# wyhuai/DDNM

Measured on AMD Instinct MI355X. Metric: restored images/sec @256×256, 100 DDIM steps, 4×SR; 1/2/4/8 GPU, higher is better.
Workload: dtype f32 (3x3 convolutions: fp32 operands carried as hi + lo fp16 halves, three fp16 MFMA products per product, fp32 accumulate -- operand error 2^-22, measured closer to fp64 than the fp32 MFMA kernel; everything else fp32); 1 GPU; celeba_hq.yml SVD sr_bicubic 4x, sigma_y=0, eta=0.85, T_sampling=100, batch_size=8 per GPU (BASELINE configs[1]); global_batch=8, image=3x256x256, parallelism=dp1 (image sharding)

## Files before the change

### ddnm_amd/_lib.py

```python
import ctypes
import os
from ctypes import POINTER, Structure, c_char_p, c_float, c_int32, c_int64, c_uint32, c_void_p

_HERE = os.path.dirname(os.path.abspath(__file__))
LIB_PATH = os.path.join(_HERE, "libddnm_hip.so")

c_f32p = c_void_p


class ConvDesc(Structure):
    _fields_ = [
        ("src0", c_void_p), ("src1", c_void_p), ("weight", c_void_p), ("bias", c_void_p),
        ("badd", c_void_p), ("res", c_void_p), ("gn_scale", c_void_p), ("gn_shift", c_void_p),
        ("out", c_void_p),
        ("B", c_int32), ("Hin", c_int32), ("Win", c_int32),
        ("C0", c_int32), ("C1", c_int32), ("Cout", c_int32),
        ("ksize", c_int32), ("stride", c_int32), ("pad", c_int32),
        ("Ho", c_int32), ("Wo", c_int32),
        ("ups", c_int32), ("gn_silu", c_int32), ("out_nchw", c_int32),
        ("badd_stride", c_int32), ("tile", c_int32),
        ("workspace", c_void_p), ("workspace_floats", c_int64),
        ("res_ups", c_int32), ("src_f16", c_int32),
        ("stats_out", c_void_p),
        ("skip0", c_void_p), ("skip1", c_void_p), ("skip_weight", c_void_p),
# ... 39 lines not shown
    _fields_ = [("sqrt_1m_at", c_float), ("sqrt_at", c_float), ("sqrt_at_next", c_float),
                ("c1", c_float), ("c2", c_float), ("lam", c_float),
                ("rng_on", c_uint32), ("rng_seed_lo", c_uint32), ("rng_seed_hi", c_uint32), ("rng_iter", c_uint32),
                ("rng_image_base", c_uint32), ("reserved_rng", c_uint32)]


PROTOTYPES = {
    "ddnm_version": (c_int32, []),
    "ddnm_error_string": (c_char_p, [c_int32]),
    "ddnm_build_digest": (c_char_p, []),
    "ddnm_sizeof": (c_int32, [c_int32]),
    "ddnm_conv2d_f32": (c_int32, [POINTER(ConvDesc), c_void_p]),
    "ddnm_conv3x3_small_cout_f32": (c_int32, [POINTER(ConvDesc), c_void_p]),
    "ddnm_conv3x3_small_cout_f32_supported": (c_int32, [POINTER(ConvDesc)]),
    "ddnm_conv2d_f32_tile_n": (c_int32, [POINTER(ConvDesc)]),
    "ddnm_conv2d_f32_workspace_floats": (c_int64, [POINTER(ConvDesc)]),
    "ddnm_conv2d_f32_stats_tiles": (c_int32, [POINTER(ConvDesc)]),
    "ddnm_conv2d_f32_fuses_skip": (c_int32, [POINTER(ConvDesc)]),
    "ddnm_spectral_mix_f32": (c_int32, [c_void_p, c_void_p, c_void_p, c_int64, c_void_p, c_int64, c_float, c_float, c_float,
                                        c_float, c_int32, c_void_p]),
    "ddnm_hq_x0_f32": (c_int32, [c_void_p, c_void_p, c_int64, c_void_p, c_int32, c_int64, c_float, c_float, c_int32,
                                 c_void_p]),
    "ddnm_hq_project_f32": (c_int32, [c_void_p, c_void_p, c_void_p, c_void_p, c_int64, c_float, c_void_p]),
    "ddnm_copy_rect_f32": (c_int32, [c_void_p, c_int32, c_int32, c_int32, c_int32, c_void_p, c_int32, c_int32, c_int32,
                                     c_int32, c_int32, c_int32, c_int32, c_void_p]),
    "ddnm_hq_sample_f32": (c_int32, [c_void_p, c_void_p, c_void_p, c_void_p, c_void_p, c_int64, c_float, c_float, c_float,
                                     c_float, c_void_p]),
    "ddnm_patchify_f32": (c_int32, [c_void_p, c_void_p, c_int32, c_int32, c_int32, c_int32, c_void_p]),
    "ddnm_im2col3x3_f16": (c_int32, [c_void_p, c_void_p, c_void_p, c_void_p, c_void_p, c_int32, c_int32, c_int32, c_int32,
                                     c_int32, c_int32, c_void_p]),
    "ddnm_gn_apply_f16": (c_int32, [c_void_p, c_void_p, c_void_p, c_void_p, c_void_p, c_int32, c_int32, c_int32, c_int32,
                                    c_int32, c_void_p]),
    "ddnm_gn_finalize_tiles_f32": (c_int32, [c_void_p, c_int32, c_int32, c_void_p, c_int32, c_int32, c_void_p, c_void_p,
                                             c_int32, c_int32, c_int32, c_float, c_void_p, c_void_p, c_void_p, c_int32,
                                             c_void_p, c_void_p]),
    "ddnm_gn_finalize_tiles_amax_f32": (c_int32, [c_void_p, c_int32, c_int32, c_void_p, c_int32, c_int32, c_void_p, c_void_p,
                                                  c_int32, c_int32, c_int32, c_float, c_void_p, c_void_p, c_void_p, c_int32,
                                                  c_void_p, c_void_p, c_void_p]),
    "ddnm_amax_bound_f32": (c_int32, [c_void_p, c_int64, c_int32, c_void_p, c_int64, c_int32, c_void_p, c_int32, c_void_p]),
    "ddnm_conv3x3_f16_f32": (c_int32, [POINTER(ConvDesc), c_void_p]),
    "ddnm_conv3x3_f16_supported": (c_int32, [POINTER(ConvDesc)]),
    "ddnm_conv3x3_f16_workspace_floats": (c_int64, [POINTER(ConvDesc)]),
    "ddnm_conv3x3_f16_stats_tiles": (c_int32, [POINTER(ConvDesc)]),
    "ddnm_conv3x3_s16_f32": (c_int32, [POINTER(ConvDesc), c_void_p]),
    "ddnm_conv3x3_s16_supported": (c_int32, [POINTER(ConvDesc)]),
    "ddnm_conv3x3_s16_persistent": (c_int32, [POINTER(ConvDesc)]),
    "ddnm_conv3x3_s16_workspace_floats": (c_int64, [POINTER(ConvDesc)]),
    "ddnm_conv3x3_s16_stats_tiles": (c_int32, [POINTER(ConvDesc)]),
    "ddnm_conv3x3_s16_act_scale": (c_float, []),
    "ddnm_conv_gather_s16_f32": (c_int32, [POINTER(ConvDesc), c_void_p]),
    "ddnm_conv_gather_s16_supported": (c_int32, [POINTER(ConvDesc)]),
    "ddnm_conv_gather_s16_workspace_floats": (c_int64, [POINTER(ConvDesc)]),
    "ddnm_conv_gather_s16_stats_tiles": (c_int32, [POINTER(ConvDesc)]),
    "ddnm_conv16": (c_int32, [POINTER(Conv16Desc), c_void_p]),
    "ddnm_conv16_supported": (c_int32, [POINTER(Conv16Desc)]),
    "ddnm_conv16_fuses_fin": (c_int32, [POINTER(Conv16Desc)]),
    "ddnm_conv16_workspace_floats": (c_int64, [POINTER(Conv16Desc)]),
    "ddnm_conv16_stats_tiles": (c_int32, [POINTER(Conv16Desc)]),
    "ddnm_gn_apply_h16": (c_int32, [c_void_p, c_void_p, c_void_p, c_void_p, c_void_p, c_int32, c_int32, c_int32, c_int32,
                                    c_int32, c_int32, c_int32, c_void_p]),
    "ddnm_im2col3x3_h16": (c_int32, [c_void_p, c_void_p, c_void_p, c_void_p, c_void_p, c_int32, c_int32, c_int32, c_int32,
                                     c_int32, c_int32, c_void_p]),
    "ddnm_nchw_to_nhwc_h16": (c_int32, [c_void_p, c_void_p, c_int32, c_int32, c_int32, c_int32, c_void_p]),
    "ddnm_gn_stats_h16": (c_int32, [c_void_p, c_void_p, c_int32, c_int32, c_int32, c_int32, c_void_p]),
    "ddnm_attn16_d64": (c_int32, [c_void_p, c_void_p, c_int32, c_int32, c_int32, c_void_p]),
    "ddnm_conv1x1_f16_f32": (c_int32, [POINTER(ConvDesc), c_void_p]),
    "ddnm_conv1x1_f16_supported": (c_int32, [POINTER(ConvDesc)]),
    "ddnm_conv1x1_f16_workspace_floats": (c_int64, [POINTER(ConvDesc)]),
    "ddnm_conv1x1_f16_stats_tiles": (c_int32, [POINTER(ConvDesc)]),
    "ddnm_gn_stats_f32": (c_int32, [c_void_p, c_void_p, c_int32, c_int32, c_int32, c_int32, c_int32, c_void_p,
                                    c_int32, c_void_p]),
    "ddnm_gn_nchunk": (c_int32, [c_int32, c_int32]),
    "ddnm_gn_finalize_f32": (c_int32, [c_void_p, c_int32, c_void_p, c_void_p, c_int32, c_int32, c_int32, c_int32,
                                       c_float, c_void_p, c_void_p, c_void_p, c_int32, c_void_p, c_void_p]),
    "ddnm_bgemm_f32": (c_int32, [POINTER(GemmDesc), c_void_p]),
    "ddnm_gn_bwd_f32": (c_int32, [c_void_p, c_void_p, c_int32, c_void_p, c_void_p, c_void_p, c_int32, c_void_p, c_int32,
                                  c_int32, c_int32, c_int32, c_int32, c_int32, c_void_p, c_int32, c_void_p, c_void_p,
                                  c_void_p]),
    "ddnm_gn_bwd_nchunk": (c_int32, [c_int32, c_int32]),
    "ddnm_gn_bwd_h16": (c_int32, [c_void_p, c_void_p, c_int32, c_void_p, c_void_p, c_void_p, c_int32, c_void_p, c_int32,
                                  c_int32, c_int32, c_int32, c_int32, c_int32, c_void_p, c_int32, c_void_p, c_void_p,
                                  c_void_p]),
    "ddnm_pool_tokens_h16": (c_int32, [c_void_p, c_void_p, c_void_p, c_void_p, c_void_p, c_int32, c_int32, c_int32,
                                       c_void_p]),
    "ddnm_pool_tokens_bwd_h16": (c_int32, [c_void_p, c_void_p, c_int32, c_int32, c_int32, c_void_p]),
    "ddnm_attn16_d64_lse": (c_int32, [c_void_p, c_void_p, c_void_p, c_int32, c_int32, c_int32, c_void_p]),
    "ddnm_attn16_d64_bwd": (c_int32, [c_void_p, c_void_p, c_void_p, c_void_p, c_void_p, c_void_p, c_int32, c_int32,
                                      c_int32, c_void_p]),
    "ddnm_softmax_bwd_rows_f32": (c_int32, [c_void_p, c_void_p, c_int64, c_int32, c_int32, c_float, c_void_p]),
    "ddnm_pool_tokens_f32": (c_int32, [c_void_p, c_void_p, c_void_p, c_void_p, c_void_p, c_int32, c_int32, c_int32,
                                       c_void_p]),
    "ddnm_pool_attn_fwd_f32": (c_int32, [c_void_p, c_void_p, c_void_p, c_int32, c_int32, c_int32, c_int32, c_void_p]),
    "ddnm_pool_attn_bwd_f32": (c_int32, [c_void_p, c_void_p, c_void_p, c_void_p, c_int32, c_int32, c_int32, c_int32,
                                         c_void_p]),
    "ddnm_pool_tokens_bwd_f32": (c_int32, [c_void_p, c_void_p, c_int32, c_int32, c_int32, c_void_p]),
    "ddnm_logsoftmax_grad_f32": (c_int32, [c_void_p, c_void_p, c_void_p, c_int32, c_int32, c_void_p]),
    "ddnm_softmax_rows_f32": (c_int32, [c_void_p, c_int64, c_int32, c_int32, c_float, c_void_p]),
    "ddnm_linear_f32": (c_int32, [c_void_p, c_void_p, c_void_p, c_void_p, c_int32, c_int32, c_int32, c_int32,
                                  c_void_p]),
    "ddnm_timestep_embedding_f32": (c_int32, [c_void_p, c_void_p, c_void_p, c_int32, c_int32, c_int32, c_void_p]),
    "ddnm_avgpool2_nhwc_f32": (c_int32, [c_void_p, c_void_p, c_void_p, c_int32, c_void_p, c_int32, c_int32, c_int32,
                                         c_int32, c_void_p]),
    "ddnm_embedding_add_f32": (c_int32, [c_void_p, c_void_p, c_void_p, c_int32, c_int32, c_int32, c_void_p]),
    "ddnm_nchw_im2col3x3_pad_f32": (c_int32, [c_void_p, c_void_p, c_int32, c_int32, c_int32, c_int32, c_int32, c_void_p]),
    "ddnm_nchw_to_nhwc_pad_f32": (c_int32, [c_void_p, c_void_p, c_int32, c_int32, c_int32, c_int32, c_void_p]),
    "ddnm_step_x0_f32": (c_int32, [c_void_p, c_void_p, c_int64, c_void_p, c_int32, c_int64, POINTER(StepScalars),
# ... 103 lines not shown
```

### ddnm_amd/build.py

```python
import hashlib
import os
import shutil
import subprocess
import sys

HERE = os.path.dirname(os.path.abspath(__file__))
CSRC = os.path.join(HERE, "csrc")
LIB = os.path.join(HERE, "libddnm_hip.so")
STAMP = os.path.join(HERE, ".libddnm_hip.stamp")
OBJ = os.path.join(HERE, "_obj")
SOURCES = ["conv_igemm_f32.hip", "conv_igemm_f16.hip", "conv_s16_persist.hip", "conv_gather_s16.hip", "conv_small_f32.hip", "conv1x1_f16.hip", "conv16.hip", "act16.hip", "attn16.hip", "attn_d512.hip", "attn16_bwd.hip", "gemm_f32.hip", "groupnorm.hip", "misc.hip", "ddnm_step.hip", "fwht.hip", "backward.hip"]
FLAGS = ["--offload-arch=gfx950", "-O3", "-std=c++17", "-fPIC", "-shared", "-Wall", "-Wno-unused-function"]


def _hipcc():
    for c in (os.environ.get("HIPCC"), shutil.which("hipcc"), "/opt/rocm/bin/hipcc"):
        if c and os.path.exists(c):
            return c
    raise RuntimeError("hipcc not found (set HIPCC)")


def _digest():
    h = hashlib.sha256()
    for f in sorted(os.listdir(CSRC)) + ["../../include/ddnm_hip.h"]:
        with open(os.path.join(CSRC, f), "rb") as fh:
            h.update(f.encode() + fh.read())
    h.update(" ".join(FLAGS).encode())
    return h.hexdigest()


LAST_BUILD = {"compiled": False}


def build(force=False, verbose=False):
    dig = _digest()
    LAST_BUILD["compiled"] = False
    if not force and os.path.exists(LIB) and os.path.exists(STAMP) and open(STAMP).read() == dig:
        return LIB
    LAST_BUILD["compiled"] = True
    tmp = LIB + f".tmp{os.getpid()}"
    os.makedirs(OBJ, exist_ok=True)
    hh = hashlib.sha256()
    for f in sorted(os.listdir(CSRC)) + ["../../include/ddnm_hip.h"]:
        if f.endswith(".h"):
            with open(os.path.join(CSRC, f), "rb") as fh:
                hh.update(f.encode() + fh.read())
    hh.update(" ".join(FLAGS).encode())
    cflags = [f for f in FLAGS if f != "-shared"]
    jobs, objs = [], []
    for s in SOURCES:
        h = hashlib.sha256(hh.digest())
        with open(os.path.join(CSRC, s), "rb") as fh:
            h.update(fh.read())
        extra = [f'-DDDNM_BUILD_DIGEST="{dig}"'] if s == "misc.hip" else []
        h.update(" ".join(extra).encode())
        obj = os.path.join(OBJ, f"{s}.{h.hexdigest()[:16]}.o")
        objs.append(obj)
        if force or not os.path.exists(obj):
            jobs.append((s, [_hipcc()] + cflags + extra + ["-c", os.path.join(CSRC, s), "-o", obj + f".tmp{os.getpid()}"], obj))
    if jobs:
        from concurrent.futures import ThreadPoolExecutor

        def run(job):
            s, cmd, obj = job
# ... 34 lines not shown
```

### ddnm_amd/csrc/conv_common.h

```cpp
#pragma once
#include "common.h"

struct ConvArgs {
    ddnm_conv_desc d;
    int Cin, ntaps, Hs, Ws;
    int m_tiles, n_tiles;
    int tiles_x;
    int TW, TW_log2;
    int ksplit;
    float* ws;
};

static inline bool conv_sizes_addressable(const ddnm_conv_desc* d) {
    const int64_t lim = (int64_t)1 << 31;
    const int64_t out_el = (int64_t)d->B * d->Ho * d->Wo * d->Cout;
    const int64_t hs = d->ups ? d->Hin / 2 : d->Hin, ws = d->ups ? d->Win / 2 : d->Win;
    const int64_t cmax = d->C0 > d->C1 ? d->C0 : d->C1;
    const int64_t src_b = (int64_t)d->B * hs * ws * cmax * (d->src_f16 ? 2 : 4);
    const int64_t cout_pad = ((int64_t)d->Cout + 127) / 128 * 128;
    const int64_t w_b = cout_pad * d->ksize * d->ksize * ((int64_t)d->C0 + d->C1) * 4;
    const int64_t sk_el = (int64_t)d->B * d->Ho * d->Wo * (d->SC0 > d->SC1 ? d->SC0 : d->SC1);
    return out_el < lim && src_b < lim && w_b < lim && sk_el < lim;
}

bool conv3x3_s16_persist_eligible(const ConvArgs& p);
int conv3x3_s16_persist_launch(const ConvArgs& p, hipStream_t s);

struct TileMap {
    int img, ty0, tx0, th_unused, TW, TW_log2, flat_base, Wo;
    bool two_d;
    __device__ __forceinline__ void pixel(int r, int& oy, int& ox) const {
        if (two_d) {
            oy = ty0 + (r >> TW_log2);
            ox = tx0 + (r & (TW - 1));
        } else {
            const int pix = flat_base + r;
            oy = pix / Wo;
            ox = pix - oy * Wo;
        }
    }
};

template <int BM>
__device__ __forceinline__ TileMap make_tilemap(const ConvArgs& p, int m_tile) {
    TileMap t;
    const int HWo = p.d.Ho * p.d.Wo;
    const int per_img = HWo / BM;
    t.img = m_tile / per_img;
    const int t_in_img = m_tile - t.img * per_img;
    t.TW = p.TW;
    t.TW_log2 = p.TW_log2;
    t.Wo = p.d.Wo;
    t.two_d = p.tiles_x != 0;
    if (t.two_d) {
        const int ty = t_in_img / p.tiles_x, tx = t_in_img - ty * p.tiles_x;
        t.ty0 = ty * (BM >> p.TW_log2);
        t.tx0 = tx << p.TW_log2;
        t.flat_base = 0;
    } else {
        t.ty0 = t.tx0 = 0;
        t.flat_base = t_in_img * BM;
    }
    return t;
}

template <int WM, int WN, int MT, int NT, bool RES_ALL_UPFRONT = false>
__device__ __forceinline__ void conv_epilogue(const ConvArgs& p, const TileMap& tm, int n_tile, int m_tile, int slice,
                                              f32x16 (&acc)[MT][NT], float* lds, const float acc_scale = 1.f) {
    constexpr int BN = WN * NT * 32;
    const ddnm_conv_desc& d = p.d;
    const int lane = threadIdx.x & 63, wave = threadIdx.x >> 6;
    const int wm = wave / WN, wn = wave % WN;
    const int ncol = lane & 31, rsel = 4 * (lane >> 5);
    const bool partial = p.ksplit > 1;
    float* __restrict__ ws = partial ? p.ws + (size_t)slice * d.B * d.Ho * d.Wo * d.Cout : nullptr;
    const float* __restrict__ res = d.res;
    float* __restrict__ out = d.out;
    const bool want_stats = d.stats_out != nullptr && !partial;
    float cs[NT], cq[NT];
// ... 261 lines not shown
```

### ddnm_amd/csrc/conv_gather_s16.hip

```cpp
#include "conv_common.h"

constexpr int GS_KC = 32;
constexpr int GS_LDH = 72;

template <int WM, int WN, int MT, int NT>
__global__ __launch_bounds__(256) void conv_gather_s16_kernel(const ConvArgs p) {
    constexpr int BM = WM * MT * 32, BN = WN * NT * 32;
    constexpr int AR = BM / 32, BR = BN / 32;
    constexpr int NWB = 3;
    constexpr int WTILE = BN * 128;
    __shared__ __attribute__((aligned(1024))) char lds_all[NWB * WTILE + BM * GS_LDH * 2];
    char* const Bs = lds_all;
    _Float16* const As = reinterpret_cast<_Float16*>(lds_all + NWB * WTILE);

    const ddnm_conv_desc& d = p.d;
    const int tid = threadIdx.x, lane = tid & 63, wave = tid >> 6;
    const int wm = wave / WN, wn = wave % WN;
    const int tile_id = xcd_swizzle(blockIdx.x, gridDim.x);
    const int n_tile = tile_id % p.n_tiles, m_tile = tile_id / p.n_tiles;
    const int slice = blockIdx.y;
    const TileMap tm = make_tilemap<BM>(p, m_tile);
    const int img = tm.img;
    float ascale, inv_ascale;
    s16_operand_scale(d.gn_scale == nullptr ? d.amax_in : nullptr, img, false, ascale, inv_ascale);
// ... 134 lines not shown
            step(it + 1, a_st1, gsc1, gsh1, a_valid1);
        }
        if (it < it_end) step(it, a_st0, gsc0, gsh0, a_valid0);
        asm volatile("s_waitcnt vmcnt(0)" ::: "memory");
    }
    __syncthreads();
    conv_epilogue<WM, WN, MT, NT>(p, tm, n_tile, m_tile, slice, acc, reinterpret_cast<float*>(As), d.acc_scale * inv_ascale);
}

struct PlanGS {
    int tile;
    int BM, BN, ksplit;
};

static bool plan_gs(const ddnm_conv_desc* d, PlanGS* pl) {
    const int HWo = d->Ho * d->Wo;
    const int Cin = d->C0 + d->C1;
    if ((d->ksize != 1 && d->ksize != 3) || (d->stride != 1 && d->stride != 2)) return false;
    if (d->C0 <= 0 || d->C0 % GS_KC || d->C1 % GS_KC || d->out_nchw || d->src_f16 || d->skip0) return false;
    if (d->Cout % 64 || HWo % 64) return false;
    {
        const int64_t px = (int64_t)d->B * (d->ups ? d->Hin / 2 : d->Hin) * (d->ups ? d->Win / 2 : d->Win);
        const int64_t cmax = d->C0 > d->C1 ? d->C0 : d->C1;
        if (px * cmax * 4 >= (int64_t)1 << 31) return false;
    }
    const int nchunks = Cin / GS_KC;
    int tile = 2;
    if (HWo % 128 == 0 && d->Cout % 128 == 0) {
        const long tiles = (long)d->B * (HWo / 128) * (d->Cout / 128);
        if (tiles * nchunks >= 256) tile = 1;
    }
    pl->tile = tile;
    pl->BM = pl->BN = tile == 1 ? 128 : 64;
    const long tiles = (long)d->B * (HWo / pl->BM) * (d->Cout / pl->BN);
    int ks = 1;
    if (d->Cout % 4 == 0 && tiles < 192) {
        ks = (int)((512 + tiles - 1) / tiles);
        if (ks > nchunks) ks = nchunks;
        if (ks > 16) ks = 16;
        if (ks < 1) ks = 1;
    }
    pl->ksplit = ks;
    return true;
}

extern "C" int ddnm_conv_gather_s16_supported(const ddnm_conv_desc* d) {
    PlanGS pl;
    return d && plan_gs(d, &pl) ? 1 : 0;
}

extern "C" int64_t ddnm_conv_gather_s16_workspace_floats(const ddnm_conv_desc* d) {
    PlanGS pl;
    if (!d || !plan_gs(d, &pl)) return DDNM_E_SHAPE;
    return pl.ksplit > 1 ? (int64_t)pl.ksplit * d->B * d->Ho * d->Wo * d->Cout : 0;
}

extern "C" int ddnm_conv_gather_s16_stats_tiles(const ddnm_conv_desc* d) {
    PlanGS pl;
    if (!d || !plan_gs(d, &pl)) return DDNM_E_SHAPE;
    return pl.ksplit > 1 ? splitk_stats_tiles(d) : d->Ho * d->Wo / pl.BM;
}

extern "C" int ddnm_conv_gather_s16_f32(const ddnm_conv_desc* d, void* stream) {
    if (!d || !d->src0 || !d->weight || !d->out) return DDNM_E_BADARG;
    if (d->B <= 0 || d->Cout <= 0 || d->Ho <= 0 || d->Wo <= 0) return DDNM_E_BADARG;
    if (!conv_sizes_addressable(d)) return DDNM_E_SHAPE;
    if (d->C1 > 0 && !d->src1) return DDNM_E_BADARG;
    if (d->gn_scale && !d->gn_shift) return DDNM_E_BADARG;
    if (!(d->acc_scale > 0.f)) return DDNM_E_BADARG;
    if (!d->gn_scale && !d->amax_in) return DDNM_E_BADARG;
    if (d->ups && ((d->Hin | d->Win) & 1)) return DDNM_E_SHAPE;
    if (d->res_ups && ((d->Ho | d->Wo) & 1)) return DDNM_E_SHAPE;
    PlanGS pl;
    if (!plan_gs(d, &pl)) return DDNM_E_SHAPE;
    if (pl.ksplit > 1) {
        const int64_t need = (int64_t)pl.ksplit * d->B * d->Ho * d->Wo * d->Cout;
        if (!d->workspace || d->workspace_floats < need) {
            if (d->stats_out) return DDNM_E_BADARG;
            pl.ksplit = 1;
        }
    }
    ConvArgs p;
    p.d = *d;
    p.Cin = d->C0 + d->C1;
    p.ntaps = d->ksize * d->ksize;
    p.Hs = d->ups ? d->Hin / 2 : d->Hin;
    p.Ws = d->ups ? d->Win / 2 : d->Win;
    p.m_tiles = d->B * (d->Ho * d->Wo / pl.BM);
    p.n_tiles = d->Cout / pl.BN;
    p.TW = 32;
    p.TW_log2 = 5;
    p.tiles_x = 0;
    p.ksplit = pl.ksplit;
    p.ws = d->workspace;
    const dim3 grid(p.m_tiles * p.n_tiles, pl.ksplit);
    hipStream_t s = (hipStream_t)stream;
    if (pl.tile == 1) { DDNM_LAUNCH((conv_gather_s16_kernel<2, 2, 2, 2>), grid, dim3(256), 0, s, p); }
    else { DDNM_LAUNCH((conv_gather_s16_kernel<2, 2, 1, 1>), grid, dim3(256), 0, s, p); }
    if (pl.ksplit > 1) return launch_splitk_reduce(p, s);
    return 0;
}
```

### ddnm_amd/ops.py

```python
import ctypes

import numpy as np
import torch

from . import _lib
from ._lib import Conv16Desc, ConvDesc, GemmDesc, StepScalars, check


def _p(t):
    return None if t is None else t.data_ptr()


def _stream():
    return torch.cuda.current_stream().cuda_stream


def _f32c(t, name):
    if t.dtype != torch.float32 or not t.is_contiguous() or not t.is_cuda:
        raise ValueError(f"{name}: expected a contiguous float32 device tensor, got {t.dtype} "
                         f"contiguous={t.is_contiguous()} device={t.device}")
    return t


class KernelTimer:
# ... 80 lines not shown


def _shape_desc(B, H, W, cin, cout, ksize=3, stride=1):
    d = ConvDesc()
    d.B, d.Hin, d.Win, d.C0, d.C1, d.Cout = B, H, W, cin, 0, cout
    d.ksize, d.stride, d.pad, d.Ho, d.Wo = ksize, stride, (ksize // 2 if stride == 1 else 0), H // stride, W // stride
    return d


def conv_fuses_skip(B, H, W, cin, cout):
    return _lib.lib().ddnm_conv2d_f32_fuses_skip(ctypes.byref(_shape_desc(B, H, W, cin, cout))) == 1


def pack_skip_weight(w, f16=False):
    p = pack_conv_weight(w).reshape(-1, w.shape[1]).contiguous()
    return p.to(torch.float16) if f16 else p


def pack_conv_weight_f16(w, cin_pad=None):
    return pack_conv_weight(w, cin_pad=cin_pad).to(torch.float16).contiguous()


def s16_weight_scale(*ws):
    import math
    m = max(float(w.abs().max()) for w in ws)
    if not (m > 0.0) or not math.isfinite(m):
        return 1.0
    return 2.0 ** (13 - math.floor(math.log2(m)))


def pack_conv_weight_s16(w, scale):
    p = pack_conv_weight(w) * float(scale)
    cp, taps, cin = p.shape
    if cin % 32:
        raise ValueError("split packing needs Cin % 32 == 0")
    hi = p.to(torch.float16)
    lo = (p - hi.float()).to(torch.float16)
    hi, lo = hi.view(cp, taps, cin // 32, 1, 32), lo.view(cp, taps, cin // 32, 1, 32)
    return torch.cat([hi, lo], 3).contiguous()


def conv_runs_s16(B, H, W, cin, cout, ups=False):
    return _lib.lib().ddnm_conv3x3_s16_supported(ctypes.byref(_shape_desc(B, H, W, cin, cout))) == 1


def conv_runs_s16_gather(B, H, W, cin, cout, ksize=3, stride=1):
    if _NO_S16_GATHER:
        return False
    return _lib.lib().ddnm_conv_gather_s16_supported(ctypes.byref(_shape_desc(B, H, W, cin, cout, ksize, stride))) == 1


_S16_ACT_SCALE = None
_NO_S16_GATHER = False


def _s16_act_scale():
    global _S16_ACT_SCALE
    if _S16_ACT_SCALE is None:
        _S16_ACT_SCALE = float(_lib.lib().ddnm_conv3x3_s16_act_scale())
    return _S16_ACT_SCALE


def conv_runs_f16(B, H, W, cin, cout, ksize=3):
    L = _lib.lib()
    d = _shape_desc(B, H, W, cin, cout, ksize)
    return (L.ddnm_conv3x3_f16_supported if ksize == 3 else L.ddnm_conv1x1_f16_supported)(ctypes.byref(d)) == 1


_F16_PREPASS_MIN_COUT = 256
_f16_scratch_buf = {}


def _f16_scratch(device, numel, slot=0):
    key = (device, slot, _stream())
    buf = _f16_scratch_buf.get(key)
    if buf is None or buf.numel() < numel:
        buf = torch.empty(numel, dtype=torch.float16, device=device)
        _f16_scratch_buf[key] = buf
    return buf


AMAX_N = 32
_S16_CHECK = False


def amax_bound(a0, a1=None):
    def src(a):
        if a is None:
            return None, 0, 0
        if isinstance(a, Act) and a.stats is not None:
            B = a.t.shape[0]
            return a.stats, a.stats.numel() // B, 1
        t = tensor_of(a)
        return _f32c(t, "amax source"), t.numel() // t.shape[0], 0
    t0 = tensor_of(a0)
    B = t0.shape[0]
    p0, n0, k0 = src(a0)
    p1, n1, k1 = src(a1)
    out = torch.empty(B * AMAX_N, dtype=torch.float32, device=t0.device)
    check(_lib.lib().ddnm_amax_bound_f32(_p(p0), n0, k0, _p(p1), n1, k1, _p(out), B, _stream()), "ddnm_amax_bound_f32")
    return out


def conv2d(src0, weight, cout, ksize, *, src1=None, bias=None, badd=None, badd_stride=0, res=None, res_ups=False,
           gn=None, gn_silu=True, stride=1, pad=None, ups=False, out=None, out_nchw=False, out_hw=None, tile=0,
           emit_stats=False, weight_f16=None, skip=None, skip_weight=None, skip_weight_f16=None, weight_s16=None,
           raw_amax=None, one_tile=False):
    a_src0, a_src1 = src0, src1
    src0, src1, res = tensor_of(src0), tensor_of(src1), tensor_of(res)
    B, Hs, Ws, C0 = src0.shape
    C1 = 0 if src1 is None else src1.shape[3]
    Hin, Win = (2 * Hs, 2 * Ws) if ups else (Hs, Ws)
    if pad is None:
        pad = ksize // 2
    if out_hw is None:
        Ho, Wo = (Hin // stride, Win // stride)
    else:
        Ho, Wo = out_hw
    if out is None:
        shape = (B, cout, Ho, Wo) if out_nchw else (B, Ho, Wo, cout)
        out = torch.empty(shape, dtype=torch.float32, device=src0.device)
    d = ConvDesc()
    d.src0, d.src1, d.weight = _p(_f32c(src0, "src0")), _p(src1), _p(_f32c(weight, "weight"))
    d.bias, d.badd, d.res = _p(bias), _p(badd), _p(res)
    d.gn_scale, d.gn_shift = (None, None) if gn is None else (_p(gn[0]), _p(gn[1]))
    d.out = _p(out)
    d.B, d.Hin, d.Win, d.C0, d.C1, d.Cout = B, Hin, Win, C0, C1, cout
    d.ksize, d.stride, d.pad, d.Ho, d.Wo = ksize, stride, pad, Ho, Wo
    d.ups, d.gn_silu, d.out_nchw = int(ups), int(gn_silu), int(out_nchw)
    d.badd_stride, d.tile, d.res_ups = badd_stride, tile, int(res_ups)
    d.flags = 1 if (one_tile or FORCE_ONE_TILE) else 0
    L = _lib.lib()
    if out_nchw and cout <= 4 and skip is None and weight_f16 is None and L.ddnm_conv3x3_small_cout_f32_supported(ctypes.byref(d)) == 1:
        _launch(L.ddnm_conv3x3_small_cout_f32, d, "ddnm_conv3x3_small_cout_f32",
                lambda: ("conv3x3_small_cout_f32", 2.0 * B * Ho * Wo * cout * 9 * C0,
                         (B, Ho, Wo, C0, cout, 3, 1, 0, 0, gn is not None, False)))
        return Act(out, None, 0) if emit_stats else out
    f16, f16_1x1 = False, False
    if skip is not None:
        s0, s1 = tensor_of(skip[0]), tensor_of(skip[1])
        d.skip0, d.skip1 = _p(s0), _p(s1)
        d.SC0, d.SC1 = s0.shape[3], (0 if s1 is None else s1.shape[3])
    s16 = (weight_s16 is not None and weight_f16 is None and ksize == 3 and stride == 1
           and (skip is None or (weight_s16[2] is not None and gn is not None and d.SC0 % 32 == 0 and d.SC1 % 32 == 0))
           and L.ddnm_conv3x3_s16_supported(ctypes.byref(d)) == 1)
    s16g = (not s16 and weight_s16 is not None and weight_f16 is None and skip is None and not _NO_S16_GATHER
            and L.ddnm_conv_gather_s16_supported(ctypes.byref(d)) == 1)
    if s16 or s16g:
        d.weight = weight_s16[0].data_ptr()
        d.acc_scale = 1.0 / (float(weight_s16[1]) * _s16_act_scale())
        if gn is None or skip is not None:
            if raw_amax is None:
                raw_amax = amax_bound(*skip) if skip is not None else amax_bound(a_src0, a_src1)
            d.amax_in = raw_amax.data_ptr()
    if weight_f16 is not None:
        if ksize == 3:
            f16 = L.ddnm_conv3x3_f16_supported(ctypes.byref(d)) == 1
            if (not f16 and stride == 1 and not ups and skip is None and not out_nchw and not res_ups
                    and Hs * Ws < 256 and (C0 | C1) % 8 == 0):
                d.ksize, d.pad, d.C0, d.C1, d.gn_scale, d.gn_shift = 1, 0, 9 * (C0 + C1), 0, None, None
                if L.ddnm_conv1x1_f16_supported(ctypes.byref(d)) == 1:
                    col = _f16_scratch(src0.device, B * Hs * Ws * 9 * (C0 + C1), slot=1)
                    check(L.ddnm_im2col3x3_f16(_p(src0), _p(src1), None if gn is None else _p(gn[0]),
                                               None if gn is None else _p(gn[1]), col.data_ptr(), B, Hs, Ws, C0, C1,
                                               int(gn_silu), _stream()), "ddnm_im2col3x3_f16")
                    d.src0, d.src1, d.src_f16 = col.data_ptr(), None, 1
                    f16 = f16_1x1 = True
                    gn = None
                else:
                    d.ksize, d.pad, d.C0, d.C1 = 3, pad, C0, C1
                    d.gn_scale, d.gn_shift = (None, None) if gn is None else (_p(gn[0]), _p(gn[1]))
        elif ksize == 1 and skip is None:
            d.gn_scale, d.gn_shift = None, None
            f16 = f16_1x1 = L.ddnm_conv1x1_f16_supported(ctypes.byref(d)) == 1
            if not f16 and gn is not None:
                d.gn_scale, d.gn_shift = _p(gn[0]), _p(gn[1])
    if f16:
        d.weight = weight_f16.data_ptr()
        if gn is not None and (f16_1x1 or cout >= _F16_PREPASS_MIN_COUT):
            h16 = _f16_scratch(src0.device, B * Hs * Ws * (C0 + C1))
            check(L.ddnm_gn_apply_f16(_p(src0), _p(src1), _p(gn[0]), _p(gn[1]), h16.data_ptr(), B, Hs * Ws, C0, C1,
                                      int(gn_silu), _stream()), "ddnm_gn_apply_f16")
            d.src0, d.src1, d.C0, d.C1 = h16.data_ptr(), None, C0 + C1, 0
            d.gn_scale, d.gn_shift, d.src_f16 = None, None, 1
    if skip is not None:
        d.skip_weight = _p(skip_weight_f16) if f16 else (weight_s16[2].data_ptr() if s16 else _p(skip_weight))
        if f16 and skip_weight_f16 is None:
            raise ValueError("fp16 launch with a fused shortcut needs skip_weight_f16")
    if f16_1x1:
        fn_run, fn_tiles, fn_ws = L.ddnm_conv1x1_f16_f32, L.ddnm_conv1x1_f16_stats_tiles, L.ddnm_conv1x1_f16_workspace_floats
    elif f16:
        fn_run, fn_tiles, fn_ws = L.ddnm_conv3x3_f16_f32, L.ddnm_conv3x3_f16_stats_tiles, L.ddnm_conv3x3_f16_workspace_floats
    elif s16:
        fn_run, fn_tiles, fn_ws = L.ddnm_conv3x3_s16_f32, L.ddnm_conv3x3_s16_stats_tiles, L.ddnm_conv3x3_s16_workspace_floats
    elif s16g:
        fn_run, fn_tiles, fn_ws = (L.ddnm_conv_gather_s16_f32, L.ddnm_conv_gather_s16_stats_tiles,
                                   L.ddnm_conv_gather_s16_workspace_floats)
    else:
        fn_run, fn_tiles, fn_ws = L.ddnm_conv2d_f32, L.ddnm_conv2d_f32_stats_tiles, L.ddnm_conv2d_f32_workspace_floats
    stats, tiles = None, 0
    if emit_stats and not _NO_FUSED_GN:
        tiles = fn_tiles(ctypes.byref(d))
        if tiles > 0:
            stats = torch.empty(B * tiles * cout * 2, dtype=torch.float32, device=src0.device)
            d.stats_out = stats.data_ptr()
    need = fn_ws(ctypes.byref(d))
    if need > 0:
        ws = _conv_workspace(src0.device, need)
        d.workspace, d.workspace_floats = ws.data_ptr(), ws.numel()

    def record():
        if f16_1x1:
            variant = "conv1x1_f16<256x128>"
        elif f16:
            variant = "conv3x3_halo_f16<256x128>"
        elif s16:
            variant = "conv3x3_s16_persist<256x128>" if L.ddnm_conv3x3_s16_persistent(ctypes.byref(d)) == 1 else "conv3x3_halo_s16<256x128>"
        elif s16g:
            variant = "conv_gather_s16"
        else:
            tn = L.ddnm_conv2d_f32_tile_n(ctypes.byref(d))
            kind = "conv3x3_halo_f32" if (ksize == 3 and stride == 1) else "conv_gather_f32"
            variant = kind + {128: "<128x128>", 64: "<64x64>", 32: "<128x32>"}[tn]
        flops = 2.0 * B * Ho * Wo * cout * (ksize * ksize * (C0 + C1) + d.SC0 + d.SC1)
        return variant, flops, (B, Ho, Wo, C0 + C1, cout, ksize, stride, int(ups), d.SC0 + d.SC1, gn is not None,
                                res is not None)
    _launch(fn_run, d, "ddnm_conv2d", record)
    if _S16_CHECK and (s16 or s16g) and not bool(torch.isfinite(out).all()):
        raise FloatingPointError(f"split-fp16 launch produced non-finite values (B={B}, {Hin}x{Win}, Cin={C0 + C1}, "
                                 f"Cout={cout}, k={ksize}): an operand left fp16 range; DDNM_CONV_F32=mfma32 selects the "
                                 "all-fp32 engine")
    if emit_stats:
        return Act(out, stats, tiles)
    return out


CONV16_COUT_ALIGN = 256


def _f16c(t, name):
    if t.dtype != torch.float16 or not t.is_contiguous() or not t.is_cuda:
        raise ValueError(f"{name}: expected a contiguous float16 device tensor, got {t.dtype} "
                         f"contiguous={t.is_contiguous()} device={t.device}")
    return t


def pack_conv_weight16(w, cin_pad=None):
    if w.dim() == 2:
        w = w[:, :, None, None]
    cout, cin, kh, kw = w.shape
    cin_pad = cin if cin_pad is None else cin_pad
    cout_pad = (cout + CONV16_COUT_ALIGN - 1) // CONV16_COUT_ALIGN * CONV16_COUT_ALIGN
    out = torch.zeros(cout_pad, kh * kw, cin_pad, dtype=torch.float16, device=w.device)
    out[:cout, :, :cin] = w.float().permute(0, 2, 3, 1).reshape(cout, kh * kw, cin).to(torch.float16)
    return out.contiguous()


def _conv16_desc(src, weight, cout, ksize, H, W, ups, skip, skip_weight, bias, res, res_ups, src1=None, gn=None,
                 gn_silu=True):
    B = src.shape[0]
    d = Conv16Desc()
    d.src, d.weight, d.bias, d.res = _p(_f16c(src, "src")), _p(_f16c(weight, "weight")), _p(bias), _p(res)
    cin = src.shape[-1]
    if src1 is not None:
        d.src1, d.C0 = _p(_f16c(src1, "src1")), cin
        cin += src1.shape[-1]
    if gn is not None:
        d.gn_scale, d.gn_shift, d.gn_silu = _p(gn[0]), _p(gn[1]), int(gn_silu)
    d.B, d.H, d.W, d.Cin, d.Cout, d.ksize = B, H, W, cin, cout, ksize
    d.ups, d.res_ups = int(ups), int(res_ups)
    if skip is not None:
        s0, s1 = skip
# ... 425 lines not shown
```

### include/ddnm_hip.h

```cpp
#ifndef DDNM_HIP_H
#define DDNM_HIP_H

#include <stdint.h>

#ifdef __cplusplus
extern "C" {
#endif

#define DDNM_E_BADARG (-1)
#define DDNM_E_SHAPE (-2)

int ddnm_version(void);
const char* ddnm_build_digest(void);
int ddnm_sizeof(int which);
const char* ddnm_error_string(int code);

typedef struct ddnm_conv_desc {
    const float* src0;
    const float* src1;
    const float* weight;
    const float* bias;
    const float* badd;
    const float* res;
    const float* gn_scale;
    const float* gn_shift;
    float* out;
    int32_t B, Hin, Win;
    int32_t C0, C1;
    int32_t Cout;
    int32_t ksize;
    int32_t stride;
    int32_t pad;
    int32_t Ho, Wo;
    int32_t ups;
    int32_t gn_silu;
    int32_t out_nchw;
    int32_t badd_stride;
    int32_t tile;
    float* workspace;
    int64_t workspace_floats;
    int32_t res_ups;
    int32_t src_f16;
    float* stats_out;
    const float* skip0;
    const float* skip1;
    const float* skip_weight;
    int32_t SC0, SC1;
    float acc_scale;
    int32_t flags;
    const float* amax_in;
} ddnm_conv_desc;

#define DDNM_CONV_ONE_TILE 1
#define DDNM_AMAX_N 32

int ddnm_conv2d_f32(const ddnm_conv_desc* d, void* stream);
int ddnm_conv2d_f32_tile_n(const ddnm_conv_desc* d);
int64_t ddnm_conv2d_f32_workspace_floats(const ddnm_conv_desc* d);
int ddnm_conv2d_f32_stats_tiles(const ddnm_conv_desc* d);
int ddnm_conv2d_f32_fuses_skip(const ddnm_conv_desc* d);

int ddnm_conv3x3_small_cout_f32(const ddnm_conv_desc* d, void* stream);
int ddnm_conv3x3_small_cout_f32_supported(const ddnm_conv_desc* d);

int ddnm_conv3x3_f16_f32(const ddnm_conv_desc* d, void* stream);
int ddnm_conv3x3_f16_supported(const ddnm_conv_desc* d);
int64_t ddnm_conv3x3_f16_workspace_floats(const ddnm_conv_desc* d);
int ddnm_conv3x3_f16_stats_tiles(const ddnm_conv_desc* d);

int ddnm_conv3x3_s16_f32(const ddnm_conv_desc* d, void* stream);
int ddnm_conv3x3_s16_supported(const ddnm_conv_desc* d);
int ddnm_conv3x3_s16_persistent(const ddnm_conv_desc* d);
int64_t ddnm_conv3x3_s16_workspace_floats(const ddnm_conv_desc* d);
int ddnm_conv3x3_s16_stats_tiles(const ddnm_conv_desc* d);
float ddnm_conv3x3_s16_act_scale(void);

int ddnm_conv_gather_s16_f32(const ddnm_conv_desc* d, void* stream);
int ddnm_conv_gather_s16_supported(const ddnm_conv_desc* d);
int64_t ddnm_conv_gather_s16_workspace_floats(const ddnm_conv_desc* d);
int ddnm_conv_gather_s16_stats_tiles(const ddnm_conv_desc* d);

int ddnm_conv1x1_f16_f32(const ddnm_conv_desc* d, void* stream);
int ddnm_conv1x1_f16_supported(const ddnm_conv_desc* d);
int64_t ddnm_conv1x1_f16_workspace_floats(const ddnm_conv_desc* d);
int ddnm_conv1x1_f16_stats_tiles(const ddnm_conv_desc* d);

typedef struct ddnm_conv16_desc {
    const void* src;
    const void* weight;
    const float* bias;
    const void* res;
    const void* skip0;
    const void* skip1;
    const void* skip_weight;
    void* out;
    float* stats_out;
    float* workspace;
    int64_t workspace_floats;
    int32_t B, H, W;
    int32_t Cin, Cout;
    int32_t ksize;
    int32_t ups, res_ups;
    int32_t SC0, SC1;
    const void* src1;
    const float* gn_scale;
    const float* gn_shift;
    int32_t C0;
    int32_t gn_silu;
    int32_t out_nchw_f32;
    int32_t reserved;
    const float* fin_gamma;
    const float* fin_beta;
    const float* fin_film;
    float* fin_scale;
    float* fin_shift;
    float fin_eps;
    int32_t fin_film_stride;
    int32_t fin_groups;
    int32_t reserved2;
} ddnm_conv16_desc;

int ddnm_conv16(const ddnm_conv16_desc* d, void* stream);
int ddnm_conv16_fuses_fin(const ddnm_conv16_desc* d);
int ddnm_conv16_supported(const ddnm_conv16_desc* d);
int64_t ddnm_conv16_workspace_floats(const ddnm_conv16_desc* d);
int ddnm_conv16_stats_tiles(const ddnm_conv16_desc* d);

int ddnm_gn_apply_h16(const void* src0, const void* src1, const float* scale, const float* shift, void* out, int32_t B,
                      int32_t H, int32_t W, int32_t C0, int32_t C1, int32_t silu, int32_t pool, void* stream);
int ddnm_im2col3x3_h16(const void* src0, const void* src1, const float* scale, const float* shift, void* out, int32_t B,
                       int32_t H, int32_t W, int32_t C0, int32_t C1, int32_t silu, void* stream);
int ddnm_nchw_to_nhwc_h16(const float* x, void* out, int32_t B, int32_t C, int32_t HW, int32_t cpad, void* stream);
int ddnm_gn_stats_h16(const void* src, float* stats, int32_t B, int32_t HW, int32_t C, int32_t tiles, void* stream);
// ... 198 lines not shown
```

Before: 6.048 images/sec.

## Add dedicated split-fp16 conv kernel for 8x8 low-resolution 3x3 layers

Adds a specialized kernel for 3x3 stride-1 convolutions at 8x8 spatial size that holds one or two whole images as the M tile, with a padded halo in LDS. All nine tap weight tiles are streamed into LDS via buffer-to-LDS loads and pipelined per tap, and a planner picks the split-K factor to fill about 256 workgroups. The generic gather path is meant to underuse the GPU and reload inputs per tap at these tiny shapes. It adds LDS pressure and a split-K reduce pass, and keeps a legacy flag to fall back.

After: 6.100 images/sec (median of 6 runs). No clear change (+0.9%).

```diff
diff --git a/ddnm_amd/_lib.py b/ddnm_amd/_lib.py
--- a/ddnm_amd/_lib.py
+++ b/ddnm_amd/_lib.py
@@ -115,6 +115,7 @@
     "ddnm_conv_gather_s16_supported": (c_int32, [POINTER(ConvDesc)]),
     "ddnm_conv_gather_s16_workspace_floats": (c_int64, [POINTER(ConvDesc)]),
     "ddnm_conv_gather_s16_stats_tiles": (c_int32, [POINTER(ConvDesc)]),
+    "ddnm_conv_lowres_s16": (c_int32, [POINTER(ConvDesc)]),
     "ddnm_conv16": (c_int32, [POINTER(Conv16Desc), c_void_p]),
     "ddnm_conv16_supported": (c_int32, [POINTER(Conv16Desc)]),
     "ddnm_conv16_fuses_fin": (c_int32, [POINTER(Conv16Desc)]),
diff --git a/ddnm_amd/build.py b/ddnm_amd/build.py
--- a/ddnm_amd/build.py
+++ b/ddnm_amd/build.py
@@ -9,7 +9,7 @@
 LIB = os.path.join(HERE, "libddnm_hip.so")
 STAMP = os.path.join(HERE, ".libddnm_hip.stamp")
 OBJ = os.path.join(HERE, "_obj")
-SOURCES = ["conv_igemm_f32.hip", "conv_igemm_f16.hip", "conv_s16_persist.hip", "conv_gather_s16.hip", "conv_small_f32.hip", "conv1x1_f16.hip", "conv16.hip", "act16.hip", "attn16.hip", "attn_d512.hip", "attn16_bwd.hip", "gemm_f32.hip", "groupnorm.hip", "misc.hip", "ddnm_step.hip", "fwht.hip", "backward.hip"]
+SOURCES = ["conv_igemm_f32.hip", "conv_igemm_f16.hip", "conv_s16_persist.hip", "conv_gather_s16.hip", "conv_lowres_s16.hip", "conv_small_f32.hip", "conv1x1_f16.hip", "conv16.hip", "act16.hip", "attn16.hip", "attn_d512.hip", "attn16_bwd.hip", "gemm_f32.hip", "groupnorm.hip", "misc.hip", "ddnm_step.hip", "fwht.hip", "backward.hip"]
 FLAGS = ["--offload-arch=gfx950", "-O3", "-std=c++17", "-fPIC", "-shared", "-Wall", "-Wno-unused-function"]
 
 
diff --git a/ddnm_amd/csrc/conv_common.h b/ddnm_amd/csrc/conv_common.h
--- a/ddnm_amd/csrc/conv_common.h
+++ b/ddnm_amd/csrc/conv_common.h
@@ -25,6 +25,9 @@
 
 bool conv3x3_s16_persist_eligible(const ConvArgs& p);
 int conv3x3_s16_persist_launch(const ConvArgs& p, hipStream_t s);
+
+bool conv_lowres_s16_plan(const ddnm_conv_desc* d, int* ksplit);
+int conv_lowres_s16_launch(const ddnm_conv_desc* d, hipStream_t s);
 
 struct TileMap {
     int img, ty0, tx0, th_unused, TW, TW_log2, flat_base, Wo;
diff --git a/ddnm_amd/csrc/conv_gather_s16.hip b/ddnm_amd/csrc/conv_gather_s16.hip
--- a/ddnm_amd/csrc/conv_gather_s16.hip
+++ b/ddnm_amd/csrc/conv_gather_s16.hip
@@ -210,12 +210,14 @@
 extern "C" int64_t ddnm_conv_gather_s16_workspace_floats(const ddnm_conv_desc* d) {
     PlanGS pl;
     if (!d || !plan_gs(d, &pl)) return DDNM_E_SHAPE;
+    conv_lowres_s16_plan(d, &pl.ksplit);
     return pl.ksplit > 1 ? (int64_t)pl.ksplit * d->B * d->Ho * d->Wo * d->Cout : 0;
 }
 
 extern "C" int ddnm_conv_gather_s16_stats_tiles(const ddnm_conv_desc* d) {
     PlanGS pl;
     if (!d || !plan_gs(d, &pl)) return DDNM_E_SHAPE;
+    if (conv_lowres_s16_plan(d, &pl.ksplit)) pl.BM = 64;
     return pl.ksplit > 1 ? splitk_stats_tiles(d) : d->Ho * d->Wo / pl.BM;
 }
 
@@ -231,6 +233,7 @@
     if (d->res_ups && ((d->Ho | d->Wo) & 1)) return DDNM_E_SHAPE;
     PlanGS pl;
     if (!plan_gs(d, &pl)) return DDNM_E_SHAPE;
+    if (conv_lowres_s16_plan(d, nullptr)) return conv_lowres_s16_launch(d, (hipStream_t)stream);
     if (pl.ksplit > 1) {
         const int64_t need = (int64_t)pl.ksplit * d->B * d->Ho * d->Wo * d->Cout;
         if (!d->workspace || d->workspace_floats < need) {
diff --git a/ddnm_amd/csrc/conv_lowres_s16.hip b/ddnm_amd/csrc/conv_lowres_s16.hip
--- /dev/null
+++ b/ddnm_amd/csrc/conv_lowres_s16.hip
@@ -0,0 +1,253 @@
+#include <type_traits>
+
+#include "conv_common.h"
+
+constexpr int LR_KC = 32;
+constexpr int LR_LDH = 72;
+constexpr int LR_BN = 64;
+constexpr int LR_WTILE = LR_BN * 128;
+constexpr int LR_HROWS = 100;
+constexpr int LR_KS_PREF = 8;
+#ifndef LR_SLICE_MAJOR
+#define LR_SLICE_MAJOR 1
+#endif
+constexpr int LR_WGS = 256;
+
+template <int IMGS>
+__global__ __launch_bounds__(256) void conv_lowres_s16_kernel(const ConvArgs p) {
+    constexpr int WM = 2, WN = 2, MT = IMGS, NT = 1;
+    constexpr int BM = 64 * IMGS;
+    constexpr int AR = BM / 32;
+    constexpr int NA = AR + 2 * IMGS;
+    constexpr int BR = LR_BN / 32;
+    constexpr int WAIT_W = 7 * BR;
+    constexpr int ABYTES = IMGS * LR_HROWS * LR_LDH * 2;
+    static_assert(IMGS == 1 || IMGS == 2, "an M tile is one or two whole images");
+    __shared__ __attribute__((aligned(1024))) char lds_all[9 * LR_WTILE + ABYTES];
+    char* const Bs = lds_all;
+    _Float16* const As = reinterpret_cast<_Float16*>(lds_all + 9 * LR_WTILE);
+
+    const ddnm_conv_desc& d = p.d;
+    const int tid = threadIdx.x, lane = tid & 63, wave = tid >> 6;
+    const int wm = wave / WN, wn = wave % WN;
+    const int tiles_mn = p.m_tiles * p.n_tiles;
+    int slice, n_tile, m_tile;
+    if (LR_SLICE_MAJOR) {
+        const int q = xcd_swizzle(blockIdx.x, gridDim.x);
+        slice = q / tiles_mn;
+        const int tile_id = q - slice * tiles_mn;
+        const bool wmajor = p.m_tiles <= 8;
+        n_tile = wmajor ? tile_id / p.m_tiles : tile_id % p.n_tiles;
+        m_tile = wmajor ? tile_id % p.m_tiles : tile_id / p.n_tiles;
+    } else {
+        slice = blockIdx.x / tiles_mn;
+        const int tile_id = xcd_swizzle(blockIdx.x - slice * tiles_mn, tiles_mn);
+        n_tile = tile_id % p.n_tiles;
+        m_tile = tile_id / p.n_tiles;
+    }
+    const int img0 = m_tile * IMGS;
+    float ascale, inv_ascale;
+    s16_operand_scale(d.gn_scale == nullptr ? d.amax_in : nullptr, img0, false, ascale, inv_ascale);
+
+    const int lrow = lane >> 3, lpiece = lane & 7;
+    const int wswz = (((wave & 1) << 2) | (lrow >> 1));
+    const unsigned w_rowlen = 9u * (unsigned)p.Cin * 4u;
+    const int cout_pad = (d.Cout + 127) / 128 * 128;
+    const __amdgpu_buffer_rsrc_t r_w = __builtin_amdgcn_make_buffer_rsrc(
+        const_cast<void*>(reinterpret_cast<const void*>(d.weight)), 0, (unsigned)cout_pad * w_rowlen, 0x00020000);
+    const unsigned w_voff = (unsigned)(n_tile * LR_BN + wave * 8 + lrow) * w_rowlen + (unsigned)((lpiece ^ wswz) * 16);
+    auto issue_w = [&](int chunk, int tap) {
+        char* dst = Bs + tap * LR_WTILE + wave * 1024;
+        const unsigned so = ((unsigned)tap * p.Cin + (unsigned)chunk * LR_KC) * 4u;
+#pragma unroll
+        for (int j = 0; j < BR; ++j)
+            __builtin_amdgcn_raw_ptr_buffer_load_lds(r_w, (__attribute__((address_space(3))) void*)(dst + j * 4096), 16, w_voff,
+                                                     so + (unsigned)j * 32u * w_rowlen, 0, 0);
+    };
+
+    const int c4 = tid & 7, row0 = tid >> 3;
+    const bool has_gn = d.gn_scale != nullptr;
+    const __amdgpu_buffer_rsrc_t r_s0 = __builtin_amdgcn_make_buffer_rsrc(
+        const_cast<float*>(d.src0), 0, (unsigned)d.B * 64u * d.C0 * 4u, 0x00020000);
+    const __amdgpu_buffer_rsrc_t r_s1 = __builtin_amdgcn_make_buffer_rsrc(
+        const_cast<float*>(d.C1 > 0 ? d.src1 : d.src0), 0, (unsigned)d.B * 64u * (d.C1 > 0 ? d.C1 : d.C0) * 4u, 0x00020000);
+    const float* const gn_sc = has_gn ? d.gn_scale + (size_t)img0 * p.Cin + c4 * 4 : reinterpret_cast<const float*>(d.weight);
+    const float* const gn_sh = has_gn ? d.gn_shift + (size_t)img0 * p.Cin + c4 * 4 : reinterpret_cast<const float*>(d.weight);
+    const int gn_img = has_gn ? p.Cin : 0;
+    const unsigned a_pix = (unsigned)(img0 * 64 + row0);
+    f32x4 a_st[AR], gsc[IMGS], gsh[IMGS];
+    auto prefetch_a = [&](int chunk) {
+        const int cb = chunk * LR_KC;
+        const bool first = cb < d.C0;
+        const unsigned cs = first ? d.C0 : d.C1, coff = first ? cb : cb - d.C0;
+        const __amdgpu_buffer_rsrc_t r_s = first ? r_s0 : r_s1;
+#pragma unroll
+        for (int i = 0; i < AR; ++i)
+            a_st[i] = __builtin_bit_cast(f32x4, __builtin_amdgcn_raw_buffer_load_b128(r_s, ((a_pix + 32u * i) * cs + c4 * 4) * 4u, coff * 4u, 0));
+#pragma unroll
+        for (int il = 0; il < IMGS; ++il) {
+            gsc[il] = *reinterpret_cast<const f32x4*>(gn_sc + il * gn_img + (has_gn ? cb : 0));
+            gsh[il] = *reinterpret_cast<const f32x4*>(gn_sh + il * gn_img + (has_gn ? cb : 0));
+        }
+    };
+    _Float16* const a_dst = As + (((row0 >> 3) + 1) * 10 + (row0 & 7) + 1) * LR_LDH + c4 * 4;
+    auto stage_a = [&]() {
+#pragma unroll
+        for (int i = 0; i < AR; ++i) {
+            f32x4 v = a_st[i];
+            if (has_gn) v = gn_act(v, gsc[i >> 1], gsh[i >> 1], d.gn_silu);
+            split_store(a_dst + ((i >> 1) * LR_HROWS + (i & 1) * 40) * LR_LDH, v, ascale);
+        }
+    };
+
+    f32x16 acc[MT][NT];
+#pragma unroll
+    for (int i = 0; i < MT; ++i)
+#pragma unroll
+        for (int r = 0; r < 16; ++r) acc[i][0][r] = 0.f;
+
+    const int nchunks = p.Cin / LR_KC;
+    const int c_begin = (int)((long)nchunks * slice / p.ksplit), c_end = (int)((long)nchunks * (slice + 1) / p.ksplit);
+    const int fr = wm * MT * 32 + (lane & 31);
+    const _Float16* const a_frag = As + ((fr >> 6) * LR_HROWS + ((fr & 63) >> 3) * 10 + (fr & 7)) * LR_LDH + (lane >> 5) * 8;
+    const int b_frag = ((wn * NT * 32 + (lane & 31)) * 128) + ((((lane >> 5) ^ (((lane & 31) >> 1) & 7))) << 4);
+
+    if (c_begin < c_end) {
+        for (int k = tid; k < ABYTES / 16; k += 256) reinterpret_cast<uint4*>(As)[k] = make_uint4(0u, 0u, 0u, 0u);
+        __builtin_amdgcn_sched_barrier(0);
+        prefetch_a(c_begin);
+        __builtin_amdgcn_sched_barrier(0);
+#pragma unroll
+        for (int t = 0; t < 8; ++t) issue_w(c_begin, t);
+        __builtin_amdgcn_sched_barrier(0);
+
+        for (int c = c_begin; c < c_end; ++c) {
+            const int cn = c + 1 < c_end ? c + 1 : c_end - 1;
+            auto tap = [&](auto T) {
+                constexpr int t = decltype(T)::value;
+                asm volatile("s_waitcnt vmcnt(%0) lgkmcnt(0)" ::"n"(t == 0 ? WAIT_W : WAIT_W + NA) : "memory");
+                __builtin_amdgcn_s_barrier();
+                asm volatile("" ::: "memory");
+                if constexpr (t == 0) {
+                    issue_w(c, 8);
+                    prefetch_a(cn);
+                } else {
+                    issue_w(cn, t - 1);
+                }
+                __builtin_amdgcn_sched_barrier(0);
+                const char* bf = Bs + t * LR_WTILE;
+                const _Float16* af = a_frag + ((t / 3) * 10 + (t % 3)) * LR_LDH;
+#pragma unroll
+                for (int ks = 0; ks < 2; ++ks) {
+                    half8 ah[MT], al[MT];
+#pragma unroll
+                    for (int i = 0; i < MT; ++i) {
+                        ah[i] = *reinterpret_cast<const half8*>(af + i * 40 * LR_LDH + ks * 16);
+                        al[i] = *reinterpret_cast<const half8*>(af + i * 40 * LR_LDH + ks * 16 + 32);
+                    }
+                    const half8 bh = *reinterpret_cast<const half8*>(bf + (b_frag ^ (ks << 5)));
+                    const half8 bl = *reinterpret_cast<const half8*>(bf + (b_frag ^ ((ks + 2) << 5)));
+#pragma unroll
+                    for (int i = 0; i < MT; ++i) acc[i][0] = __builtin_amdgcn_mfma_f32_32x32x16_f16(al[i], bh, acc[i][0], 0, 0, 0);
+#pragma unroll
+                    for (int i = 0; i < MT; ++i) acc[i][0] = __builtin_amdgcn_mfma_f32_32x32x16_f16(ah[i], bl, acc[i][0], 0, 0, 0);
+#pragma unroll
+                    for (int i = 0; i < MT; ++i) acc[i][0] = __builtin_amdgcn_mfma_f32_32x32x16_f16(ah[i], bh, acc[i][0], 0, 0, 0);
+                }
+            };
+            asm volatile("s_waitcnt lgkmcnt(0)" ::: "memory");
+            __builtin_amdgcn_s_barrier();
+            asm volatile("s_waitcnt vmcnt(%0)" ::"n"(8 * BR) : "memory");
+            stage_a();
+            tap(std::integral_constant<int, 0>{});
+            tap(std::integral_constant<int, 1>{});
+            tap(std::integral_constant<int, 2>{});
+            tap(std::integral_constant<int, 3>{});
+            tap(std::integral_constant<int, 4>{});
+            tap(std::integral_constant<int, 5>{});
+            tap(std::integral_constant<int, 6>{});
+            tap(std::integral_constant<int, 7>{});
+            tap(std::integral_constant<int, 8>{});
+        }
+        asm volatile("s_waitcnt vmcnt(0)" ::: "memory");
+    }
+    __syncthreads();
+    TileMap tm;
+    tm.img = img0;
+    tm.ty0 = tm.tx0 = tm.th_unused = 0;
+    tm.TW = p.TW;
+    tm.TW_log2 = p.TW_log2;
+    tm.flat_base = 0;
+    tm.Wo = d.Wo;
+    tm.two_d = false;
+    conv_epilogue<WM, WN, MT, NT>(p, tm, n_tile, m_tile, slice, acc, reinterpret_cast<float*>(As), d.acc_scale * inv_ascale);
+}
+
+struct PlanLR {
+    int imgs, ksplit;
+};
+
+static bool plan_lr(const ddnm_conv_desc* d, PlanLR* pl) {
+    if (d->flags & DDNM_CONV_LEGACY_GATHER) return false;
+    if (d->ksize != 3 || d->stride != 1 || d->pad != 1) return false;
+    if (d->Ho != 8 || d->Wo != 8 || d->Hin != 8 || d->Win != 8 || d->ups || d->res_ups) return false;
+    if (d->C0 <= 0 || d->C0 % LR_KC || d->C1 % LR_KC || d->Cout % LR_BN) return false;
+    if (d->out_nchw || d->src_f16 || d->skip0 || d->B <= 0) return false;
+    const int nchunks = (d->C0 + d->C1) / LR_KC;
+    const long n_tiles = d->Cout / LR_BN;
+    int imgs = 1;
+    if (d->gn_scale && d->B % 2 == 0 && (d->B / 2) * n_tiles * LR_KS_PREF >= LR_WGS) imgs = 2;
+    long tiles = (d->B / imgs) * n_tiles;
+    int ks = (int)(LR_WGS / tiles);
+    if (ks > nchunks) ks = nchunks;
+    if (ks > 16) ks = 16;
+    if (ks <= 1 || d->Cout % 4) {
+        ks = 1;
+        imgs = 1;
+    }
+    pl->imgs = imgs;
+    pl->ksplit = ks;
+    return true;
+}
+
+bool conv_lowres_s16_plan(const ddnm_conv_desc* d, int* ksplit) {
+    PlanLR pl;
+    if (!plan_lr(d, &pl)) return false;
+    if (ksplit) *ksplit = pl.ksplit;
+    return true;
+}
+
+int conv_lowres_s16_launch(const ddnm_conv_desc* d, hipStream_t s) {
+    PlanLR pl;
+    if (!plan_lr(d, &pl)) return DDNM_E_SHAPE;
+    if (pl.ksplit > 1) {
+        const int64_t need = (int64_t)pl.ksplit * d->B * 64 * d->Cout;
+        if (!d->workspace || d->workspace_floats < need) {
+            if (d->stats_out) return DDNM_E_BADARG;
+            pl.ksplit = 1;
+            pl.imgs = 1;
+        }
+    }
+    ConvArgs p;
+    p.d = *d;
+    p.Cin = d->C0 + d->C1;
+    p.ntaps = 9;
+    p.Hs = p.Ws = 8;
+    p.m_tiles = d->B / pl.imgs;
+    p.n_tiles = d->Cout / LR_BN;
+    p.TW = 32;
+    p.TW_log2 = 5;
+    p.tiles_x = 0;
+    p.ksplit = pl.ksplit;
+    p.ws = d->workspace;
+    const dim3 grid(p.m_tiles * p.n_tiles * pl.ksplit);
+    if (pl.imgs == 2) { DDNM_LAUNCH((conv_lowres_s16_kernel<2>), grid, dim3(256), 0, s, p); }
+    else { DDNM_LAUNCH((conv_lowres_s16_kernel<1>), grid, dim3(256), 0, s, p); }
+    if (pl.ksplit > 1) return launch_splitk_reduce(p, s);
+    return 0;
+}
+
+extern "C" int ddnm_conv_lowres_s16(const ddnm_conv_desc* d) {
+    PlanLR pl;
+    return d && plan_lr(d, &pl) ? 1 : 0;
+}
diff --git a/ddnm_amd/ops.py b/ddnm_amd/ops.py
--- a/ddnm_amd/ops.py
+++ b/ddnm_amd/ops.py
@@ -156,6 +156,7 @@
 
 _S16_ACT_SCALE = None
 _NO_S16_GATHER = False
+LEGACY_GATHER = _os.environ.get("DDNM_LOWRES", "") == "legacy"
 
 
 def _s16_act_scale():
@@ -209,7 +210,7 @@
 def conv2d(src0, weight, cout, ksize, *, src1=None, bias=None, badd=None, badd_stride=0, res=None, res_ups=False,
            gn=None, gn_silu=True, stride=1, pad=None, ups=False, out=None, out_nchw=False, out_hw=None, tile=0,
            emit_stats=False, weight_f16=None, skip=None, skip_weight=None, skip_weight_f16=None, weight_s16=None,
-           raw_amax=None, one_tile=False):
+           raw_amax=None, one_tile=False, legacy_gather=False):
     a_src0, a_src1 = src0, src1
     src0, src1, res = tensor_of(src0), tensor_of(src1), tensor_of(res)
     B, Hs, Ws, C0 = src0.shape
@@ -233,7 +234,7 @@
     d.ksize, d.stride, d.pad, d.Ho, d.Wo = ksize, stride, pad, Ho, Wo
     d.ups, d.gn_silu, d.out_nchw = int(ups), int(gn_silu), int(out_nchw)
     d.badd_stride, d.tile, d.res_ups = badd_stride, tile, int(res_ups)
-    d.flags = 1 if (one_tile or FORCE_ONE_TILE) else 0
+    d.flags = (1 if (one_tile or FORCE_ONE_TILE) else 0) | (2 if (legacy_gather or LEGACY_GATHER) else 0)
     L = _lib.lib()
     if out_nchw and cout <= 4 and skip is None and weight_f16 is None and L.ddnm_conv3x3_small_cout_f32_supported(ctypes.byref(d)) == 1:
         _launch(L.ddnm_conv3x3_small_cout_f32, d, "ddnm_conv3x3_small_cout_f32",
@@ -321,7 +322,7 @@
         elif s16:
             variant = "conv3x3_s16_persist<256x128>" if L.ddnm_conv3x3_s16_persistent(ctypes.byref(d)) == 1 else "conv3x3_halo_s16<256x128>"
         elif s16g:
-            variant = "conv_gather_s16"
+            variant = "conv_lowres_s16" if L.ddnm_conv_lowres_s16(ctypes.byref(d)) == 1 else "conv_gather_s16"
         else:
             tn = L.ddnm_conv2d_f32_tile_n(ctypes.byref(d))
             kind = "conv3x3_halo_f32" if (ksize == 3 and stride == 1) else "conv_gather_f32"
diff --git a/include/ddnm_hip.h b/include/ddnm_hip.h
--- a/include/ddnm_hip.h
+++ b/include/ddnm_hip.h
@@ -52,6 +52,7 @@
 } ddnm_conv_desc;
 
 #define DDNM_CONV_ONE_TILE 1
+#define DDNM_CONV_LEGACY_GATHER 2
 #define DDNM_AMAX_N 32
 
 int ddnm_conv2d_f32(const ddnm_conv_desc* d, void* stream);
@@ -79,6 +80,7 @@
 int ddnm_conv_gather_s16_supported(const ddnm_conv_desc* d);
 int64_t ddnm_conv_gather_s16_workspace_floats(const ddnm_conv_desc* d);
 int ddnm_conv_gather_s16_stats_tiles(const ddnm_conv_desc* d);
+int ddnm_conv_lowres_s16(const ddnm_conv_desc* d);
 
 int ddnm_conv1x1_f16_f32(const ddnm_conv_desc* d, void* stream);
 int ddnm_conv1x1_f16_supported(const ddnm_conv_desc* d);
```
